# daxiongpro/EPNet

Measured on AMD Instinct MI355X. Metric: SA-stack points/sec per GPU (16384-pt KITTI scene) + % HBM roofline, higher is better.
Workload: dtype f32; 1 GPU; 256 x 16384-pt kitti scenes per GPU per step through the 4-level SA op stack (4 samplings [FPS + centre gather; levels 2-4 nested in level 1 where tie-free] + 8 ball_query + 8 fused groupings [xyz - centre ; features]), pyramid 16384>4096>1024>256>64, radii [[.1,.5],[.5,1],[1,2],[2,4]], nsample [16,32], C=0/96/256/512, HIP-graph launch; levels=4, scenes_per_gpu=256, software_pipelined=True, pipeline_stages=2, parallelism=scene-parallel x1

## Files before the change

epnet_amd/_lib.py:

```python
import ctypes
import os

_HERE = os.path.dirname(os.path.abspath(__file__))
LIB_PATH = os.environ.get("EPNET_HIP_LIB") or os.path.join(_HERE, "lib", "libepnet_hip.so")

_vp = ctypes.c_void_p
_i = ctypes.c_int
_f = ctypes.c_float
_sz = ctypes.c_size_t
_i64 = ctypes.c_int64

SIGNATURES = {
    "epnet_abi_version": (_i, []),
    "epnet_strerror": (ctypes.c_char_p, [_i]),
    "epnet_last_hip_error": (ctypes.c_char_p, []),
    "epnet_furthest_point_sampling": (_i, [_i, _i, _i, _vp, _vp, _vp, _vp]),
    "epnet_gather_points": (_i, [_i, _i, _i, _i, _vp, _vp, _vp, _vp]),
    "epnet_gather_points_grad": (_i, [_i, _i, _i, _i, _vp, _vp, _vp, _vp]),
    "epnet_ball_query": (_i, [_i, _i, _i, _f, _i, _vp, _vp, _vp, _vp]),
    "epnet_ball_query_workspace_bytes": (_sz, [_i, _i, _i]),
    "epnet_ball_query_ws": (_i, [_i, _i, _i, _f, _i, _vp, _vp, _vp, _vp, _sz, _vp]),
    "epnet_group_points": (_i, [_i, _i, _i, _i, _i, _vp, _vp, _vp, _vp]),
    "epnet_group_points_grad": (_i, [_i, _i, _i, _i, _i, _vp, _vp, _vp, _vp]),
    "epnet_group_concat": (_i, [_i, _i, _i, _i, _i, _vp, _vp, _vp, _vp, _vp, _i, _vp]),
# ... 5 lines not shown
    "epnet_group_concat_grad_ws": (_i, [_i, _i, _i, _i, _i, _vp, _vp, _vp, _i, _vp, _sz, _vp]),
    "epnet_three_nn": (_i, [_i, _i, _i, _vp, _vp, _vp, _vp, _vp]),
    "epnet_three_nn_workspace_bytes": (_sz, [_i, _i, _i]),
    "epnet_three_nn_ws": (_i, [_i, _i, _i, _vp, _vp, _vp, _vp, _vp, _sz, _vp]),
    "epnet_three_interpolate": (_i, [_i, _i, _i, _i, _vp, _vp, _vp, _vp, _vp]),
    "epnet_three_interpolate_grad": (_i, [_i, _i, _i, _i, _vp, _vp, _vp, _vp, _vp]),
    "epnet_three_interpolate_grad_workspace_bytes": (_sz, [_i, _i, _i]),
    "epnet_three_interpolate_grad_ws": (_i, [_i, _i, _i, _i, _vp, _vp, _vp, _vp, _vp, _sz, _vp]),
    "epnet_group_linear": (_i, [_i, _i, _i, _i, _i, _vp, _vp, _vp, _vp, _vp, _vp, _vp, _vp]),
    "epnet_group_linear_grad_w": (_i, [_i, _i, _i, _i, _i, _vp, _vp, _vp, _vp, _vp, _vp]),
    "epnet_feature_gather": (_i, [_i, _i, _i, _i, _i, _i, _i, _vp, _vp, _vp, _vp, _vp, _vp]),
    "epnet_feature_gather_grad": (_i, [_i, _i, _i, _i, _i, _i, _vp, _vp, _vp, _vp]),
    "epnet_pool_max": (_i, [ctypes.c_longlong, _i, _vp, _vp, _vp, _vp]),
    "epnet_pool_max_grad": (_i, [ctypes.c_longlong, _i, _vp, _vp, _vp, _vp]),
    "epnet_scene_index_bytes": (_sz, [_i, _i]),
    "epnet_scene_index_build": (_i, [_i, _i, _vp, _vp, _sz, _vp]),
    "epnet_scene_index_build_gathered": (_i, [_i, _i, _i, _vp, _vp, _vp, _vp, _sz, _vp]),
    "epnet_furthest_point_sampling_indexed": (_i, [_i, _i, _i, _vp, _vp, _sz, _vp, _vp, _vp]),
    "epnet_sample_centres": (_i, [_i, _i, _i, _vp, _vp, _sz, _vp, _vp, _vp, _vp]),
    "epnet_sample_centres_chain": (_i, [_i, _i, _i, _vp, _vp, _sz, _vp, _vp, _vp, _vp, _vp, _i, _vp]),
    "epnet_group_concat_multi": (_i, [_i, _i, _i, _i, _i, _vp, _vp, _vp, _vp, _vp, _vp, _i, _vp]),
    "epnet_ball_query_indexed_multi": (_i, [_i, _i, _i, _i, _vp, _vp, _vp, _vp, _vp, _sz, _vp, _vp]),
    "epnet_ball_query_ordered": (_i, [_i, _i, _i, _i, _vp, _vp, _vp, _vp, _vp, _sz, _vp, _sz, _vp, _vp]),
    "epnet_three_nn_indexed": (_i, [_i, _i, _i, _vp, _vp, _vp, _sz, _vp, _sz, _vp, _vp, _vp]),
    "epnet_ball_query_indexed": (_i, [_i, _i, _i, _f, _i, _vp, _vp, _vp, _sz, _vp, _vp]),
    "epnet_boxes_overlap_bev": (_i, [_i, _vp, _i, _vp, _vp, _vp]),
    "epnet_boxes_iou_bev": (_i, [_i, _vp, _i, _vp, _vp, _vp]),
    "epnet_boxes_iou3d": (_i, [_i, _vp, _i, _vp, _vp, _vp]),
    "epnet_boxes_iou3d_pairs": (_i, [_i, _vp, _vp, _vp, _vp]),
    "epnet_aug_roi_by_noise": (_i, [_i, _i, _f, _vp, _vp, _vp, _vp, _vp, _vp, _vp, _vp]),
    "epnet_rpn_proposals_workspace_bytes": (_sz, [_i, _i, _i, _i]),
    "epnet_rpn_proposals": (_i, [_i, _i, _vp, _vp, _vp, _i, _i, _i, _f, _i, _vp, _sz, _vp, _vp, _vp, _vp]),
    "epnet_nms_workspace_bytes": (_sz, [_i]),
    "epnet_nms": (_i, [_vp, _i, _f, _vp, _sz, _vp, _vp, _vp]),
    "epnet_nms_normal": (_i, [_vp, _i, _f, _vp, _sz, _vp, _vp, _vp]),
    "epnet_roipool3d_workspace_bytes": (_sz, [_i, _i, _i]),
    "epnet_roipool3d": (_i, [_i, _i, _i, _i, _i, _vp, _vp, _vp, _vp, _vp, _vp, _sz, _vp]),
    "epnet_pts_in_boxes3d_host": (_i, [_vp, _vp, _vp, _i64, _i64]),
    "epnet_roipool3d_host": (_i, [_vp, _vp, _vp, _vp, _vp, _vp, _i64, _i64, _i64, _i64]),
}

_lib = None


class EpnetError(RuntimeError):
    pass
# ... 30 lines not shown
```

epnet_amd/csrc/ball_query.hip:

```cpp
#include <stdlib.h>

#include "common.h"
#include "dpp.h"
#include "spatial.h"

namespace epnet {

constexpr int kBqTile = 2048;
constexpr int kBqThreads = 256;

template <int CPW>
__global__ __launch_bounds__(kBqThreads) void ball_query_kernel(int n, int m, float radius2, int nsample,
                                                                const float *__restrict__ new_xyz,
                                                                const float *__restrict__ xyz,
                                                                int *__restrict__ idx) {
    __shared__ float tile[kBqTile * 3];
    const int lane = threadIdx.x & 63, wave = threadIdx.x >> 6;
    const int bs = blockIdx.y;
    xyz += (size_t)bs * n * 3;
    new_xyz += (size_t)bs * m * 3;
    idx += (size_t)bs * m * nsample;

    const int c0 = (blockIdx.x * (kBqThreads / 64) + wave) * CPW;
    float cx[CPW], cy[CPW], cz[CPW];
// ... 325 lines not shown
        for (int q0 = 0; q0 < nq; q0 += 64) {
            const int qd = q0 + lane;
            const bool qnear = qd < nq && box_near(qboxes + qd * 6, cx, cy, cz, r2);
            const unsigned long long qmask = __ballot(qnear);
            if (!qmask) continue;
            const int nqc = (int)__popcll(qmask);
            if (qnear) quads[popc_below(qmask)] = qd;
            __builtin_amdgcn_wave_barrier();
            for (int s0 = 0; s0 < nqc; s0 += 16) {
                const int slot = s0 + (lane >> 2);
                int bid = 0;
                bool bnear = false;
                if (slot < nqc) {
                    bid = quads[slot] * 4 + (lane & 3);
                    bnear = box_near(boxes + bid * 6, cx, cy, cz, r2);
                }
                scan_buckets(__ballot(bnear), [&](int l) { return __builtin_amdgcn_readlane(bid, l); });
            }
            __builtin_amdgcn_wave_barrier();
        }
    }
}

__device__ __forceinline__ void bq_emit_list(int lane, const int *hits, int cnt, int nsample, int *__restrict__ out) {
    __builtin_amdgcn_wave_barrier();
    const int mine = lane < cnt ? hits[lane] : 0x7fffffff;
    int rank = 0;
    for (int j = 0; j < cnt; ++j) rank += __builtin_amdgcn_readlane(mine, j) < mine ? 1 : 0;
    if (lane < cnt && rank < nsample) out[rank] = mine;
    int first = 0;
    if (cnt) first = __builtin_amdgcn_readlane(mine, (int)__builtin_ctzll(__ballot(lane < cnt && rank == 0)));
    for (int l = cnt + lane; l < nsample; l += 64) out[l] = first;
}

template <int RM>
__device__ __forceinline__ int bq_select_smallest(int lane, int *hits, int cnt, int nsample, int np) {
    __builtin_amdgcn_wave_barrier();
    int key[RM];
#pragma unroll
    for (int r = 0; r < RM; ++r) key[r] = (r * 64 < cnt && r * 64 + lane < cnt) ? hits[r * 64 + lane] : 0x7fffffff;
    int lo = 0, hi = np;
    while (hi - lo > 1) {
        const int mid = (lo + hi) >> 1;
        int c = 0;
#pragma unroll
        for (int r = 0; r < RM; ++r)
            if (r * 64 < cnt) c += (int)__popcll(__ballot(key[r] < mid));
// ... 38 lines not shown
    if (bc > 0 && (pos < nsample || pos == 0)) {
        for (int i = 0; i < DPL; ++i) {
            unsigned ww = bits[lane * DPL + i];
            if (ww && mine_first == 0x7fffffff) mine_first = (lane * DPL + i) * 32 + (int)__builtin_ctz(ww);
            while (ww && pos < nsample) {
                const int bit = (int)__builtin_ctz(ww);
                ww &= ww - 1u;
                out[pos++] = (lane * DPL + i) * 32 + bit;
            }
            if (pos >= nsample) break;
        }
    }
    const unsigned long long have = __ballot(bc > 0);
    int first = 0;
    if (have) first = __builtin_amdgcn_readlane(mine_first, (int)__builtin_ctzll(have));
    for (int l = total + lane; l < nsample; l += 64) out[l] = first;
}

template <int K>
struct BqScales {
    float r2[K];
    int nsample[K];
    int *idx[K];
};

template <int DPL, int K>
__global__ __launch_bounds__(kQThreads) void bq_query_kernel(int np, int m, BqScales<K> sc,
                                                             const float *__restrict__ new_xyz,
                                                             const float4 *__restrict__ sorted,
                                                             const float *__restrict__ boxes,
                                                             const float *__restrict__ qboxes,
                                                             const float4 *__restrict__ order, int npc) {
    __shared__ unsigned s_bits[kQThreads / 64][64 * DPL];
    __shared__ int s_quads[kQThreads / 64][64];
    __shared__ int s_hits[kQThreads / 64][K][64];
    const int lane = threadIdx.x & 63, wave = threadIdx.x >> 6;
    int wg_x, bs;
    xcd_scene_map(wg_x, bs);
    int ci = wg_x * (kQThreads / 64) + wave;
    if (ci >= m) return;
    sorted += (size_t)bs * np;
    boxes += (size_t)bs * (np / 64) * 6;
    qboxes += (size_t)bs * (np / 256) * 6;
    float cx, cy, cz;
    if (order) {
        const float4 e = order[(size_t)bs * npc + ci];
        ci = __float_as_int(e.w);
// ... 12 lines not shown
        if (!__ballot(d2 < r2max)) return;
#pragma unroll
        for (int k = 0; k < K; ++k) {
            const bool hit = d2 < sc.r2[k];
            const unsigned long long hm = __ballot(hit);
            if (hm) {
                const int pos = cnt[k] + popc_below(hm);
                if (hit && pos < 64) s_hits[wave][k][pos] = __float_as_int(p.w);
                cnt[k] += (int)__popcll(hm);
            }
        }
    });
#pragma unroll
    for (int k = 0; k < K; ++k) {
        int *out = sc.idx[k] + ((size_t)bs * m + ci) * sc.nsample[k];
        if (cnt[k] <= 64)
            bq_emit_list(lane, s_hits[wave][k], cnt[k], sc.nsample[k], out);
        else
            bq_bitmap_search<DPL>(lane, np, sc.r2[k], sc.nsample[k], cx, cy, cz, sorted, boxes, qboxes, out, s_bits[wave],
                                  s_quads[wave]);
    }
}

template <int DPL, int K, bool kStream>
__global__ __launch_bounds__(kQThreads) void bq_query2_kernel(int np, int m, BqScales<K> sc,
                                                              const float *__restrict__ new_xyz,
                                                              const float4 *__restrict__ sorted,
                                                              const float *__restrict__ boxes,
                                                              const float *__restrict__ qboxes,
                                                              const float4 *__restrict__ order, int npc) {
    constexpr int CAP = kStream ? (K == 1 ? 512 : 256) : 64, kStepAppends = 128;
    constexpr int kBitWords = kStream ? 0 : 64 * DPL;
    __shared__ unsigned s_pool[kQThreads / 64][kBitWords + 2 * K * CAP];
    __shared__ int s_quads[kQThreads / 64][2][64];
    const int lane = threadIdx.x & 63, wave = threadIdx.x >> 6;
    int wg_x, bs;
    xcd_scene_map(wg_x, bs);
    const int ci0 = (wg_x * (kQThreads / 64) + wave) * 2;
    if (ci0 >= m) return;
    const bool two = ci0 + 1 < m;
    sorted += (size_t)bs * np;
    boxes += (size_t)bs * (np / 64) * 6;
    qboxes += (size_t)bs * (np / 256) * 6;
    float ax, ay, az, bx_, by_, bz_;
    int out0 = ci0, out1 = ci0 + 1;
    if (order) {
        const float4 e0 = order[(size_t)bs * npc + ci0], e1 = order[(size_t)bs * npc + ci0 + (two ? 1 : 0)];
        ax = e0.x; ay = e0.y; az = e0.z;
        bx_ = e1.x; by_ = e1.y; bz_ = e1.z;
        out0 = __float_as_int(e0.w);
        out1 = __float_as_int(e1.w);
    } else {
        const float *c0 = new_xyz + ((size_t)bs * m + ci0) * 3;
        const float *c1 = two ? c0 + 3 : c0;
        ax = c0[0]; ay = c0[1]; az = c0[2];
        bx_ = c1[0]; by_ = c1[1]; bz_ = c1[2];
// ... 96 lines not shown
                const int slot = s0 + ((lane & 31) >> 2);
                int bid = 0;
                bool bnear = false;
                if (slot < nmine) {
                    bid = s_quads[wave][half][slot] * 4 + (lane & 3);
                    bnear = box_near(boxes + bid * 6, hx, hy, hz, r2max);
                }
                const unsigned long long cand = __ballot(bnear);
                scan_pairs(cand & 0xFFFFFFFFull, cand >> 32,
                           [&](int e, int bit) { return __builtin_amdgcn_readlane(bid, bit + 32 * e); });
            }
            __builtin_amdgcn_wave_barrier();
        }
    }
#ifdef EPNET_BQ_STATS
    const unsigned long long st_1 = __builtin_amdgcn_s_memtime();
#endif
#pragma unroll
    for (int e = 0; e < 2; ++e) {
        if (e == 1 && !two) break;
        const float cx = e ? bx_ : ax, cy = e ? by_ : ay, cz = e ? bz_ : az;
#pragma unroll
        for (int k = 0; k < K; ++k) {
            int *out = sc.idx[k] + ((size_t)bs * m + (e ? out1 : out0)) * sc.nsample[k];
            int *hits = hits_of + (e * K + k) * CAP;
            if constexpr (kStream) {
                if (cnt[e][k] > 64) {
                    bq_select_smallest<CAP / 64>(lane, hits, cnt[e][k], sc.nsample[k], np);
                    cnt[e][k] = sc.nsample[k];
#ifdef EPNET_BQ_STATS
                    st_sel = true;
#endif
                }
                bq_emit_list(lane, hits, cnt[e][k], sc.nsample[k], out);
            } else {
                if (cnt[e][k] <= 64) {
                    bq_emit_list(lane, hits, cnt[e][k], sc.nsample[k], out);
                } else {
#ifdef EPNET_BQ_STATS
                    st_again = true;
#endif
                    bq_bitmap_search<DPL>(lane, np, sc.r2[k], sc.nsample[k], cx, cy, cz, sorted, boxes, qboxes, out, s_pool[wave],
                                          s_quads[wave][0]);
                }
            }
        }
    }
#ifdef EPNET_BQ_STATS
    {
        const unsigned long long st_3 = __builtin_amdgcn_s_memtime();
        if (lane == 0) {
            const int o = st_again ? 8 : (st_sel ? 4 : 0);
            atomicAdd(&g_bq_stats[o + 0], 1ull);
            atomicAdd(&g_bq_stats[o + 1], st_1 - st_0);
            atomicAdd(&g_bq_stats[o + 2], st_3 - st_1);
            atomicAdd(&g_bq_stats[o + 3], (unsigned long long)st_rows);
            atomicMax(&g_bq_stats[12], st_3 - st_0);
        }
    }
#endif
}

}

using namespace epnet;

extern "C" int epnet_ball_query(int b, int n, int m, float radius, int nsample, const float *new_xyz,
                                const float *xyz, int *idx, epnet_stream_t stream) {
    EPNET_REQUIRE(b >= 0 && n >= 0 && m >= 0 && nsample >= 0);
// ... 10 lines not shown
        dim3 grid(div_up(m, waves), b);
        hipLaunchKernelGGL(ball_query_kernel<1>, grid, dim3(kBqThreads), 0, s, n, m, radius2, nsample, new_xyz, xyz, idx);
    }
    return check_launch("ball_query");
}


int epnet::spatial_index_launch(int b, int n, int np, const float *xyz, float4 *sorted, float *boxes, float *qboxes,
                                hipStream_t s, int n_src, const int *src_idx, float *gathered) {
    if (n <= 4096) {
        constexpr int T = 256, cells = 1 << 12;
        const size_t stage = (np & 255) == 0 ? (size_t)(np / 4 < 512 ? np / 4 : 512) * sizeof(float4) : 0;
        hipLaunchKernelGGL((bq_index_kernel<T, 12>), dim3(b), dim3(T), (size_t)(cells + cells / (cells / T) + 64) * sizeof(int) + stage, s,
                           n, np, xyz, sorted, boxes, qboxes, n_src, src_idx, gathered);
    } else {
        constexpr int T = 1024, cells = 1 << 14;
        const size_t stage = (n <= T * 16 && (np & 255) == 0) ? (size_t)(np / 4) * sizeof(float4) : 0;
        hipLaunchKernelGGL((bq_index_kernel<T, 14>), dim3(b), dim3(T), (size_t)(cells + cells / (cells / T) + 64) * sizeof(int) + stage, s,
                           n, np, xyz, sorted, boxes, qboxes, n_src, src_idx, gathered);
    }
    return check_launch("spatial index");
}

template <int K>
static int bq_query_launch(int b, int np, int m, const BqScales<K> &sc, const float *new_xyz, const float4 *sorted,
                           hipStream_t s, const float4 *order = nullptr, int npc = 0) {
    const float *boxes = (const float *)(sorted + (size_t)b * np);
    const float *qboxes = boxes + (size_t)b * (np / 64) * 6;
    const char *pair_str = getenv("EPNET_BQ_PAIR");
    const int pair_env = pair_str ? atoi(pair_str) : -1;
    const bool pair = pair_env >= 0 ? pair_env != 0 : (long long)b * m >= 65536;
    const char *pad_str = getenv("EPNET_BQ_PAD_KB");
    const size_t pad = pad_str ? (size_t)atoi(pad_str) * 1024 : 0;
    if (pair) {
        dim3 grid(div_up(div_up(m, 2), kQThreads / 64), b);
        bool stream = np > 16384;
        if (const char *e = getenv("EPNET_BQ_STREAM")) stream = atoi(e) != 0;
        for (int k = 0; k < K; ++k) stream = stream && sc.nsample[k] <= 64;
#define EPNET_BQ2(D_)                                                                                                                   \
    do {                                                                                                                                \
        if (stream)                                                                                                                     \
            hipLaunchKernelGGL((bq_query2_kernel<D_, K, true>), grid, dim3(kQThreads), pad, s, np, m, sc, new_xyz, sorted, boxes, qboxes, \
                               order, npc);                                                                                             \
        else                                                                                                                            \
            hipLaunchKernelGGL((bq_query2_kernel<D_, K, false>), grid, dim3(kQThreads), pad, s, np, m, sc, new_xyz, sorted, boxes,       \
                               qboxes, order, npc);                                                                                     \
    } while (0)
        switch (np / 2048) {
            case 1: EPNET_BQ2(1); break;
            case 2: EPNET_BQ2(2); break;
            case 4: EPNET_BQ2(4); break;
            case 8: EPNET_BQ2(8); break;
            case 16: EPNET_BQ2(16); break;
            default: EPNET_BQ2(32); break;
        }
#undef EPNET_BQ2
        return check_launch("ball_query query");
    }
    dim3 grid(div_up(m, kQThreads / 64), b);
#define EPNET_BQ(D_) hipLaunchKernelGGL((bq_query_kernel<D_, K>), grid, dim3(kQThreads), pad, s, np, m, sc, new_xyz, sorted, boxes, qboxes, order, npc)
    switch (np / 2048) {
        case 1: EPNET_BQ(1); break;
        case 2: EPNET_BQ(2); break;
        case 4: EPNET_BQ(4); break;
        case 8: EPNET_BQ(8); break;
        case 16: EPNET_BQ(16); break;
        default: EPNET_BQ(32); break;
    }
#undef EPNET_BQ
    return check_launch("ball_query query");
}

extern "C" size_t epnet_scene_index_bytes(int b, int n) { return scene_index_bytes(b, n); }

extern "C" int epnet_scene_index_build(int b, int n, const float *xyz, void *index, size_t index_bytes,
                                       epnet_stream_t stream) {
    const size_t need = scene_index_bytes(b, n);
    EPNET_REQUIRE(need != 0 && xyz && index);
    if (index_bytes < need) return EPNET_ENOMEM;
// ... 39 lines not shown
extern "C" int epnet_ball_query_indexed_multi(int b, int n, int m, int nscales, const float *radii, const int *nsamples,
                                              const float *new_xyz, const float *xyz, const void *index,
                                              size_t index_bytes, int *const *idx, epnet_stream_t stream) {
    EPNET_REQUIRE(nscales >= 0 && (nscales == 0 || (radii && nsamples && idx)));
    const size_t need = scene_index_bytes(b, n);
    bool fused = nscales == 2 && need != 0 && index && m > 0 && nsamples[0] > 0 && nsamples[1] > 0;
    if (!fused) {
        for (int k = 0; k < nscales; ++k) {
            const int rc = epnet_ball_query_indexed(b, n, m, radii[k], nsamples[k], new_xyz, xyz, index, index_bytes, idx[k], stream);
            if (rc) return rc;
        }
        return EPNET_OK;
    }
    EPNET_REQUIRE(new_xyz && idx[0] && idx[1]);
    if (index_bytes < need) return EPNET_ENOMEM;
    EPNET_REQUIRE(b <= 65535);
    BqScales<2> sc;
    for (int k = 0; k < 2; ++k) {
        sc.r2[k] = radii[k] * radii[k];
        sc.nsample[k] = nsamples[k];
        sc.idx[k] = idx[k];
    }
    return bq_query_launch<2>(b, scene_index_np(n), m, sc, new_xyz, (const float4 *)index, (hipStream_t)stream);
}

extern "C" int epnet_ball_query_ordered(int b, int n, int m, int nscales, const float *radii, const int *nsamples,
                                        const float *new_xyz, const float *xyz, const void *index, size_t index_bytes,
                                        const void *centre_index, size_t centre_index_bytes, int *const *idx,
                                        epnet_stream_t stream) {
    EPNET_REQUIRE(nscales >= 0 && (nscales == 0 || (radii && nsamples && idx)));
    const size_t need = scene_index_bytes(b, n), need_c = scene_index_bytes(b, m);
    bool ordered = (nscales == 1 || nscales == 2) && need != 0 && need_c != 0 && index && centre_index && m > 0;
    for (int k = 0; ordered && k < nscales; ++k) ordered = nsamples[k] > 0 && idx[k] != nullptr;
    const char *force = getenv("EPNET_BQ_ORDERED");
    if (force ? atoi(force) == 0 : n <= 16384) ordered = false;
    if (!ordered) return epnet_ball_query_indexed_multi(b, n, m, nscales, radii, nsamples, new_xyz, xyz, index, index_bytes, idx, stream);
    if (index_bytes < need || centre_index_bytes < need_c) return EPNET_ENOMEM;
    EPNET_REQUIRE(b <= 65535);
    const int np = scene_index_np(n), npc = scene_index_np(m);
    if (nscales == 1) {
        BqScales<1> sc;
        sc.r2[0] = radii[0] * radii[0];
        sc.nsample[0] = nsamples[0];
        sc.idx[0] = idx[0];
        return bq_query_launch<1>(b, np, m, sc, new_xyz, (const float4 *)index, (hipStream_t)stream, (const float4 *)centre_index, npc);
    }
// ... 42 lines not shown
```

epnet_amd/csrc/common.h:

```cpp
#pragma once
#include <hip/hip_runtime.h>
#include <stdint.h>

#include "epnet_ops.h"

namespace epnet {

constexpr int kWave = 64;

int record_hip_error(hipError_t e, const char *where);

inline int check_launch(const char *where) {
    hipError_t e = hipGetLastError();
    if (e != hipSuccess) return record_hip_error(e, where);
    return EPNET_OK;
}

inline int div_up(int a, int b) { return (a + b - 1) / b; }
inline long long div_up64(long long a, long long b) { return (a + b - 1) / b; }

__device__ __forceinline__ int lane_id() { return threadIdx.x & (kWave - 1); }

__device__ __forceinline__ int popc_below(unsigned long long mask) {
    return __builtin_amdgcn_mbcnt_hi((unsigned)(mask >> 32), __builtin_amdgcn_mbcnt_lo((unsigned)mask, 0));
}

__device__ __forceinline__ void store_stream(float *dst, float x, float y, float z, float w) {
    typedef float f4 __attribute__((ext_vector_type(4)));
    const f4 v = {x, y, z, w};
    __builtin_nontemporal_store(v, reinterpret_cast<f4 *>(dst));
}

__device__ __forceinline__ void xcd_scene_map(int &wg_x, int &bs) {
#ifdef EPNET_NO_XCD_MAP
    wg_x = (int)blockIdx.x;
    bs = (int)blockIdx.y;
#else
    const int gx = (int)gridDim.x, nwg = gx * (int)gridDim.y, orig = (int)blockIdx.y * gx + (int)blockIdx.x;
    const int xcd = orig & 7, qq = nwg >> 3, rr = nwg & 7;
    const int wgid = (xcd < rr ? xcd * (qq + 1) : rr * (qq + 1) + (xcd - rr) * qq) + (orig >> 3);
    bs = wgid / gx;
    wg_x = wgid - bs * gx;
// ... 33 lines not shown
```

epnet_amd/csrc/group.hip:

```cpp
#include <stdlib.h>

#include "common.h"
#include "spatial.h"
#include "runsum.h"

namespace epnet {

constexpr int kGThreads = 256;
constexpr int kGChan = 16;

__global__ __launch_bounds__(kGThreads) void gather_rows_vec4_kernel(int c, int n, int p, size_t ostride,
                                                                     const float *__restrict__ points,
                                                                     const int *__restrict__ idx,
                                                                     float *__restrict__ out) {
    int wg_x, wg_y, bs;
    xcd_scene_map3(wg_x, wg_y, bs);
    const int c0 = wg_y * kGChan;
    const int q4 = wg_x * kGThreads + threadIdx.x;
    if (q4 * 4 >= p) return;
    const int4 id = *reinterpret_cast<const int4 *>(idx + (size_t)bs * p + (size_t)q4 * 4);
    const int cend = min(c, c0 + kGChan);
    const float *src = points + ((size_t)bs * c + c0) * n;
    float *dst = out + (size_t)bs * ostride + (size_t)c0 * p + (size_t)q4 * 4;
#pragma unroll 4
// ... 568 lines not shown
    return launch_gather_rows(b, c, n, npoints, points, idx, out, (hipStream_t)stream, "gather_points");
}

extern "C" int epnet_gather_points_grad(int b, int c, int n, int npoints, const float *grad_out, const int *idx,
                                        float *grad_points, epnet_stream_t stream) {
    EPNET_REQUIRE(b >= 0 && c >= 0 && n >= 0 && npoints >= 0);
    return launch_scatter_rows(b, c, n, npoints, grad_out, idx, grad_points, (hipStream_t)stream, "gather_points_grad");
}

extern "C" int epnet_group_points(int b, int c, int n, int npoints, int nsample, const float *points, const int *idx,
                                  float *out, epnet_stream_t stream) {
    EPNET_REQUIRE(b >= 0 && c >= 0 && n >= 0 && npoints >= 0 && nsample >= 0);
    return launch_gather_rows(b, c, n, (long long)npoints * nsample, points, idx, out, (hipStream_t)stream,
                              "group_points");
}

extern "C" int epnet_group_points_grad(int b, int c, int n, int npoints, int nsample, const float *grad_out,
                                       const int *idx, float *grad_points, epnet_stream_t stream) {
    EPNET_REQUIRE(b >= 0 && c >= 0 && n >= 0 && npoints >= 0 && nsample >= 0);
    return launch_scatter_rows(b, c, n, (long long)npoints * nsample, grad_out, idx, grad_points, (hipStream_t)stream,
                               "group_points_grad");
}

static int launch_group_xyz(int b, int n, int npoints, int nsample, long long p, size_t ostride, const float *xyz,
                            const float *new_xyz, const int *idx, float *out, hipStream_t s) {
    if (nsample % 4 == 0 && (((uintptr_t)idx | (uintptr_t)out) % 16 == 0) && (ostride % 4 == 0))
        hipLaunchKernelGGL(group_xyz_centred_vec4_kernel, dim3((unsigned)div_up64(p / 4, kGThreads), b), dim3(kGThreads), 0, s, n,
                           npoints, nsample, ostride, xyz, new_xyz, idx, out);
    else
        hipLaunchKernelGGL(group_xyz_centred_kernel, dim3((unsigned)div_up64(p, kGThreads), b), dim3(kGThreads), 0, s, n, npoints,
                           nsample, ostride, xyz, new_xyz, idx, out);
    return check_launch("group_concat xyz");
}

extern "C" int epnet_group_concat(int b, int c, int n, int npoints, int nsample, const float *xyz, const float *new_xyz,
                                  const float *features, const int *idx, float *out, int use_xyz, epnet_stream_t stream) {
    EPNET_REQUIRE(b >= 0 && c >= 0 && n >= 0 && npoints >= 0 && nsample >= 0);
    EPNET_REQUIRE(use_xyz || c > 0);
    const long long p = (long long)npoints * nsample;
    if (b == 0 || p == 0) return EPNET_OK;
    EPNET_REQUIRE(idx && out && (c == 0 || features) && (!use_xyz || (xyz && new_xyz)));
    EPNET_REQUIRE(n > 0);
    if (p > 0x7fffffffll || b > 65535) return EPNET_ELIMIT;
    hipStream_t s = (hipStream_t)stream;
    const int ch0 = use_xyz ? 3 : 0;
    const size_t ostride = (size_t)(ch0 + c) * (size_t)p;
    if (use_xyz) {
// ... 184 lines not shown
```

epnet_amd/pointnet2_cuda.py:

```python
import torch

from . import _lib
from ._tensor import dev_ptr, need, on_device_of, writes

_F, _I = torch.float32, torch.int32


@writes("idx")
def ball_query_wrapper(b, n, m, radius, nsample, new_xyz, xyz, idx):
    pn, px, pi = dev_ptr(new_xyz, "new_xyz", _F), dev_ptr(xyz, "xyz", _F), dev_ptr(idx, "idx", _I)
    need(new_xyz, b * m * 3, "new_xyz"); need(xyz, b * n * 3, "xyz"); need(idx, b * m * nsample, "idx")
    l = _lib.lib()
    ws_bytes = l.epnet_ball_query_workspace_bytes(b, n, m)
    with on_device_of(xyz) as s:
        if ws_bytes:
            ws = torch.empty((ws_bytes,), dtype=torch.uint8, device=xyz.device)
            _lib.check(l.epnet_ball_query_ws(b, n, m, radius, nsample, pn, px, pi, ws.data_ptr(), ws_bytes, s), "ball_query")
        else:
            _lib.check(l.epnet_ball_query(b, n, m, radius, nsample, pn, px, pi, s), "ball_query")
    return 1


@writes("out")
def group_points_wrapper(b, c, n, npoints, nsample, points, idx, out):
# ... 182 lines not shown
                       "sample_centres")
    return 1


@writes("idxs")
def ball_query_multi_wrapper(b, n, m, radii, nsamples, new_xyz, xyz, index, idxs):
    import ctypes
    pn, pxyz = dev_ptr(new_xyz, "new_xyz", _F), dev_ptr(xyz, "xyz", _F)
    need(new_xyz, b * m * 3, "new_xyz"); need(xyz, b * n * 3, "xyz")
    k = len(radii)
    assert len(nsamples) == k and len(idxs) == k
    ptrs = []
    for ns, t in zip(nsamples, idxs):
        ptrs.append(dev_ptr(t, "idx", _I))
        need(t, b * m * ns, "idx")
    px, nb = _index_args(index, xyz)
    c_r = (ctypes.c_float * k)(*[float(r) for r in radii])
    c_n = (ctypes.c_int * k)(*[int(x) for x in nsamples])
    c_p = (ctypes.c_void_p * k)(*ptrs)
    with on_device_of(xyz) as s:
        _lib.check(_lib.lib().epnet_ball_query_indexed_multi(b, n, m, k, ctypes.cast(c_r, ctypes.c_void_p),
                                                             ctypes.cast(c_n, ctypes.c_void_p), pn, pxyz, px, nb,
                                                             ctypes.cast(c_p, ctypes.c_void_p), s), "ball_query")
    return 1


@writes("idxs")
def ball_query_ordered_wrapper(b, n, m, radii, nsamples, new_xyz, xyz, index, centre_index, idxs):
    import ctypes
    pn, pxyz = dev_ptr(new_xyz, "new_xyz", _F), dev_ptr(xyz, "xyz", _F)
    need(new_xyz, b * m * 3, "new_xyz"); need(xyz, b * n * 3, "xyz")
    k = len(radii)
    assert len(nsamples) == k and len(idxs) == k
    ptrs = []
    for ns, t in zip(nsamples, idxs):
        ptrs.append(dev_ptr(t, "idx", _I))
        need(t, b * m * ns, "idx")
    px, nb = _index_args(index, xyz)
    pc, nc = _index_args(centre_index, new_xyz)
    c_r = (ctypes.c_float * k)(*[float(r) for r in radii])
    c_n = (ctypes.c_int * k)(*[int(x) for x in nsamples])
    c_p = (ctypes.c_void_p * k)(*ptrs)
    with on_device_of(xyz) as s:
        _lib.check(_lib.lib().epnet_ball_query_ordered(b, n, m, k, ctypes.cast(c_r, ctypes.c_void_p), ctypes.cast(c_n, ctypes.c_void_p),
                                                     pn, pxyz, px, nb, pc, nc, ctypes.cast(c_p, ctypes.c_void_p), s), "ball_query")
    return 1
# ... 166 lines not shown
```

epnet_amd/sa_stack.py:

```python
import os

import torch

from . import pointnet2_cuda as ext

RPN_NPOINTS = (4096, 1024, 256, 64)
RPN_RADII = ((0.1, 0.5), (0.5, 1.0), (1.0, 2.0), (2.0, 4.0))
RPN_NSAMPLES = ((16, 32), (16, 32), (16, 32), (16, 32))
RPN_FEAT_CHANNELS = (0, 96, 256, 512)
RPN_FP = ((1024, 64, 256), (512, 256, 1024), (512, 1024, 4096), (256, 4096, 16384))


CONFIGS = {
    2: dict(n=16384, npoints=RPN_NPOINTS, radii=RPN_RADII, nsamples=RPN_NSAMPLES, feat_channels=RPN_FEAT_CHANNELS),
    5: dict(n=65536, npoints=(16384,), radii=((0.5,),), nsamples=((64,),), feat_channels=(64,)),
}


def sa_algorithmic_bytes(n=16384, npoints=RPN_NPOINTS, nsamples=RPN_NSAMPLES, feat_channels=RPN_FEAT_CHANNELS):
    out = {"fps": 0, "gather": 0, "ball_query": 0, "group_xyz": 0, "group_feat": 0}
    cur = n
    for lvl, m in enumerate(npoints):
        out["fps"] += cur * 12 + m * 4
        out["gather"] += m * 4 + 3 * cur * 4 + 3 * m * 4
# ... 40 lines not shown
            chosen = frozenset(int(v) for v in s_query_levels)
        elif queries_in_s is not None:
            chosen = every if queries_in_s else frozenset()
        elif env_lv is not None:
            chosen = frozenset(int(v) for v in env_lv.split(",") if v.strip())
        elif self.stages == 3:
            chosen = every
        elif env_q == 2 or (env_q == 1 and with_fp):
            chosen = every
        elif env_q == 1 and batch * n >= 240 * 16384:
            chosen = every - {0}
        else:
            chosen = frozenset()
        self.s_query_levels = chosen & every
        self.queries_in_s = self.s_query_levels == every
        self.chain = bool(int(os.environ.get("EPNET_SA_CHAIN", "1"))) and fused_sampling
        self.fuse_gather = bool(int(os.environ.get("EPNET_SA_FUSE_GATHER", "1")))
        self._deferred = None
        self.s_first = bool(int(os.environ.get("EPNET_SA_S_FIRST", "0" if self.s_query_levels else "1")))
        self.tail_scales = int(os.environ.get("EPNET_SA_TAIL_SCALES", "0"))
        self.multi_query = bool(int(os.environ.get("EPNET_SA_MULTI_QUERY", "1")))
        self.multi_group = bool(int(os.environ.get("EPNET_SA_MULTI_GROUP", "1")))
        self.ordered_query = bool(int(os.environ.get("EPNET_SA_ORDERED_QUERY", "1")))
        self.side = None
        self.npoints, self.radii, self.nsamples, self.feat_channels = npoints, radii, nsamples, feat_channels
        self.with_fp, self.fp = with_fp, fp
        dev = torch.device(device)
        g = torch.Generator().manual_seed(seed)
        f32, i32 = torch.float32, torch.int32
        self.levels = []
        cur = n
        for lvl, m in enumerate(npoints):
            c = feat_channels[lvl]
            index_bytes = ext.scene_index_bytes(batch, cur) if shared_index else 0
            L = {
                "n": cur, "m": m, "c": c,
                "xyz_t_sets": [torch.empty((batch, 3, cur), dtype=f32, device=dev) for _ in range(self.ring if not fused else 1)],
                "temp": torch.empty((batch, cur), dtype=f32, device=dev),
                "fps_idx_sets": ([torch.empty((batch, m), dtype=i32, device=dev) for _ in range(3)] if self.stages == 3 else None),
                "fps_idx": None,
                "new_xyz_t": torch.empty((batch, 3, m), dtype=f32, device=dev),
                "sets": [{"new_xyz": torch.empty((batch, m, 3), dtype=f32, device=dev),
                          "index": (torch.empty((index_bytes,), dtype=torch.uint8, device=dev) if index_bytes else None),
                          "prefix": torch.zeros((batch,), dtype=i32, device=dev),
                          "centre_index": (torch.empty((ext.scene_index_bytes(batch, m),), dtype=torch.uint8, device=dev)
                                           if (shared_index and lvl + 1 == len(npoints) and ext.scene_index_bytes(batch, m)) else None)}
# ... 141 lines not shown
        else:
            for S in L["scales"]:
                self._query_scale(L, S, cur_xyz, parity)

    def _centre_index(self, L, parity):
        lvl = self.levels.index(L)
        if lvl + 1 < len(self.levels):
            return self.levels[lvl + 1]["sets"][parity]["index"] if self.shared_index else None
        own = L["sets"][parity].get("centre_index")
        if own is not None:
            ext.scene_index_build_wrapper(self.batch, L["m"], L["sets"][parity]["new_xyz"], own)
        return own

    def _group_scales(self, L, cur_xyz, parity):
        if self.fused and self.multi_group and len(L["scales"]) > 1:
            ext.group_concat_multi_wrapper(self.batch, L["c"], L["n"], L["m"], [S["ns"] for S in L["scales"]], cur_xyz,
                                           L["sets"][parity]["new_xyz"], L["features"], [self._idx(S, parity) for S in L["scales"]],
                                           [S["grouped"] for S in L["scales"]], True)
        else:
            for S in L["scales"]:
                self._group_scale(L, S, cur_xyz, parity)

    def _group_level(self, L, cur_xyz, parity):
        self._query_level(L, cur_xyz, parity)
        self._group_scales(L, cur_xyz, parity)

    def _side_stream(self, device):
        if self.side is None:
            self.side = torch.cuda.Stream(device=device)
        return self.side

    def run(self, xyz):
        main = torch.cuda.current_stream(xyz.device)
        side = self._side_stream(xyz.device) if self.overlap else None
        cur_xyz = xyz
        built = False
        for lvl, L in enumerate(self.levels):
            new_xyz = self._sample_level(L, cur_xyz, 0, index_built=built)
            built = False
            nxt = self.levels[lvl + 1] if lvl + 1 < len(self.levels) else None
            if self.ordered_query and L["n"] > 16384 and nxt is not None and nxt["sets"][0]["index"] is not None:
                ext.scene_index_build_wrapper(self.batch, L["m"], new_xyz, nxt["sets"][0]["index"])
                built = True
            if side is not None:
                side.wait_stream(main)
                with torch.cuda.stream(side):
# ... 209 lines not shown
```

include/epnet_ops.h:

```cpp
#ifndef EPNET_OPS_H
#define EPNET_OPS_H

#include <stddef.h>
#include <stdint.h>

#ifdef __cplusplus
extern "C" {
#endif

#define EPNET_ABI_VERSION 1

#define EPNET_OK 0
#define EPNET_EINVAL (-1)
#define EPNET_ELAUNCH (-2)
#define EPNET_ENOMEM (-3)
#define EPNET_ELIMIT (-4)

typedef void *epnet_stream_t;

int epnet_abi_version(void);
const char *epnet_strerror(int code);
const char *epnet_last_hip_error(void);


// ... 72 lines not shown
                         const float *xy, const int *idx, float *out, float *xy_out, epnet_stream_t stream);
int epnet_feature_gather_grad(int b, int c, int h, int w, int n, int align_corners, const float *grad_out, const float *xy,
                              float *grad_feature_map, epnet_stream_t stream);

size_t epnet_scene_index_bytes(int b, int n);
int epnet_scene_index_build(int b, int n, const float *xyz, void *index, size_t index_bytes, epnet_stream_t stream);
int epnet_scene_index_build_gathered(int b, int n_src, int n, const float *xyz_src, const int *idx, float *gathered, void *index,
                                     size_t index_bytes, epnet_stream_t stream);
int epnet_furthest_point_sampling_indexed(int b, int n, int m, const float *xyz, void *index,
                                          size_t index_bytes, float *temp, int *idx, epnet_stream_t stream);
int epnet_sample_centres(int b, int n, int m, const float *xyz, void *index, size_t index_bytes, float *temp,
                         int *idx, float *new_xyz, epnet_stream_t stream);
int epnet_sample_centres_chain(int b, int n, int m, const float *xyz, void *index, size_t index_bytes, float *temp,
                               int *idx, float *new_xyz, const int *prefix_in, int *prefix_out, int prefix_cap,
                               epnet_stream_t stream);
int epnet_three_nn_indexed(int b, int n, int m, const float *unknown, const float *known, const void *unknown_index,
                           size_t unknown_index_bytes, const void *known_index, size_t known_index_bytes, float *dist2,
                           int *idx, epnet_stream_t stream);
int epnet_ball_query_indexed(int b, int n, int m, float radius, int nsample, const float *new_xyz, const float *xyz,
                             const void *index, size_t index_bytes, int *idx, epnet_stream_t stream);
int epnet_ball_query_indexed_multi(int b, int n, int m, int nscales, const float *radii, const int *nsamples,
                                   const float *new_xyz, const float *xyz, const void *index, size_t index_bytes,
                                   int *const *idx, epnet_stream_t stream);
int epnet_ball_query_ordered(int b, int n, int m, int nscales, const float *radii, const int *nsamples, const float *new_xyz,
                             const float *xyz, const void *index, size_t index_bytes, const void *centre_index,
                             size_t centre_index_bytes, int *const *idx, epnet_stream_t stream);


int epnet_boxes_overlap_bev(int num_a, const float *boxes_a, int num_b, const float *boxes_b,
                            float *ans_overlap, epnet_stream_t stream);

int epnet_boxes_iou_bev(int num_a, const float *boxes_a, int num_b, const float *boxes_b,
                        float *ans_iou, epnet_stream_t stream);

int epnet_boxes_iou3d(int num_a, const float *boxes_a, int num_b, const float *boxes_b, float *ans_iou3d,
                      epnet_stream_t stream);

int epnet_boxes_iou3d_pairs(int k, const float *boxes_a, const float *boxes_b, float *ans_iou3d, epnet_stream_t stream);

int epnet_aug_roi_by_noise(int k, int aug_times, float pos_thresh, float *roi_boxes3d, const float *gt_boxes3d,
                           const float *iou3d_src, const int *tries, const unsigned char *keep_draw,
                           const float *noise, float *iou_of_rois, epnet_stream_t stream);

size_t epnet_rpn_proposals_workspace_bytes(int b, int distance_based, int pre_nms_top_n, int post_nms_top_n);
int epnet_rpn_proposals(int b, int n, const float *proposals, const float *scores, const int64_t *order,
                        int distance_based, int pre_nms_top_n, int post_nms_top_n, float nms_thresh, int rotated,
// ... 32 lines not shown
```

Before: 1.323 billion points/s.

## Fuse centred xyz grouping into the paired ball-query kernel for C=0 levels

```diff
diff --git a/epnet_amd/_lib.py b/epnet_amd/_lib.py
--- a/epnet_amd/_lib.py
+++ b/epnet_amd/_lib.py
@@ -51,6 +51,7 @@
     "epnet_group_concat_multi": (_i, [_i, _i, _i, _i, _i, _vp, _vp, _vp, _vp, _vp, _vp, _i, _vp]),
     "epnet_ball_query_indexed_multi": (_i, [_i, _i, _i, _i, _vp, _vp, _vp, _vp, _vp, _sz, _vp, _vp]),
     "epnet_ball_query_ordered": (_i, [_i, _i, _i, _i, _vp, _vp, _vp, _vp, _vp, _sz, _vp, _sz, _vp, _vp]),
+    "epnet_ball_query_group_xyz": (_i, [_i, _i, _i, _i, _vp, _vp, _vp, _vp, _vp, _sz, _i, _vp, _vp, _vp]),
     "epnet_three_nn_indexed": (_i, [_i, _i, _i, _vp, _vp, _vp, _sz, _vp, _sz, _vp, _vp, _vp]),
     "epnet_ball_query_indexed": (_i, [_i, _i, _i, _f, _i, _vp, _vp, _vp, _sz, _vp, _vp]),
     "epnet_boxes_overlap_bev": (_i, [_i, _vp, _i, _vp, _vp, _vp]),
diff --git a/epnet_amd/csrc/ball_query.hip b/epnet_amd/csrc/ball_query.hip
--- a/epnet_amd/csrc/ball_query.hip
+++ b/epnet_amd/csrc/ball_query.hip
@@ -371,7 +371,7 @@
     }
 }
 
-__device__ __forceinline__ void bq_emit_list(int lane, const int *hits, int cnt, int nsample, int *__restrict__ out) {
+__device__ __forceinline__ void bq_emit_list(int lane, const int *hits, int cnt, int nsample, int *out) {
     __builtin_amdgcn_wave_barrier();
     const int mine = lane < cnt ? hits[lane] : 0x7fffffff;
     int rank = 0;
@@ -456,7 +456,53 @@
     float r2[K];
     int nsample[K];
     int *idx[K];
+    float *grp[K];
+    unsigned long long gstride[K];
 };
+
+template <int V, int K>
+__device__ __forceinline__ void bq_write_rows(int lane, const BqScales<K> &sc, const int *hits_of, int cap, bool two, int bs, int m,
+                                              int row0, int row1, float ax, float ay, float az, float bx, float by, float bz,
+                                              const float *__restrict__ xyz, int n) {
+    const int u0 = sc.nsample[0] / V, u1 = K > 1 ? sc.nsample[K - 1] / V : 0, per_centre = u0 + u1;
+    const int total = two ? 2 * per_centre : per_centre;
+    const float *base = xyz + (size_t)bs * n * 3;
+    for (int f = lane; f < total; f += 64) {
+        int g = f;
+        const bool e = g >= per_centre;
+        g = e ? g - per_centre : g;
+        const bool k1 = K > 1 && g >= u0;
+        g = k1 ? g - u0 : g;
+        const int ns = k1 ? sc.nsample[K - 1] : sc.nsample[0];
+        int *idx = k1 ? sc.idx[K - 1] : sc.idx[0];
+        float *grp = k1 ? sc.grp[K - 1] : sc.grp[0];
+        const size_t gstride = k1 ? sc.gstride[K - 1] : sc.gstride[0];
+        const int row = e ? row1 : row0;
+        const float cx = e ? bx : ax, cy = e ? by : ay, cz = e ? bz : az;
+        const int *src = hits_of + ((e ? K : 0) + (k1 ? 1 : 0)) * cap + g * V;
+        const size_t p = (size_t)m * ns, o = (size_t)row * ns + (size_t)g * V;
+        float *dst = grp + (size_t)bs * gstride + o;
+        if constexpr (V == 4) {
+            const int4 id = *reinterpret_cast<const int4 *>(src);
+            *reinterpret_cast<int4 *>(idx + (size_t)bs * p + o) = id;
+            const float *p0 = base + (size_t)id.x * 3, *p1 = base + (size_t)id.y * 3, *p2 = base + (size_t)id.z * 3,
+                        *p3 = base + (size_t)id.w * 3;
+            const float x0 = p0[0], y0 = p0[1], z0 = p0[2], x1 = p1[0], y1 = p1[1], z1 = p1[2];
+            const float x2 = p2[0], y2 = p2[1], z2 = p2[2], x3 = p3[0], y3 = p3[1], z3 = p3[2];
+            store_stream(dst, x0 - cx, x1 - cx, x2 - cx, x3 - cx);
+            store_stream(dst + p, y0 - cy, y1 - cy, y2 - cy, y3 - cy);
+            store_stream(dst + 2 * p, z0 - cz, z1 - cz, z2 - cz, z3 - cz);
+        } else {
+            const int id = *src;
+            idx[(size_t)bs * p + o] = id;
+            const float *pt = base + (size_t)id * 3;
+            const float x = pt[0], y = pt[1], z = pt[2];
+            dst[0] = x - cx;
+            dst[p] = y - cy;
+            dst[2 * p] = z - cz;
+        }
+    }
+}
 
 template <int DPL, int K>
 __global__ __launch_bounds__(kQThreads) void bq_query_kernel(int np, int m, BqScales<K> sc,
@@ -515,16 +561,17 @@
     }
 }
 
-template <int DPL, int K, bool kStream>
+template <int DPL, int K, bool kStream, int kXyz>
 __global__ __launch_bounds__(kQThreads) void bq_query2_kernel(int np, int m, BqScales<K> sc,
                                                               const float *__restrict__ new_xyz,
                                                               const float4 *__restrict__ sorted,
                                                               const float *__restrict__ boxes,
                                                               const float *__restrict__ qboxes,
-                                                              const float4 *__restrict__ order, int npc) {
+                                                              const float4 *__restrict__ order, int npc,
+                                                              const float *__restrict__ xyz, int n) {
     constexpr int CAP = kStream ? (K == 1 ? 512 : 256) : 64, kStepAppends = 128;
     constexpr int kBitWords = kStream ? 0 : 64 * DPL;
-    __shared__ unsigned s_pool[kQThreads / 64][kBitWords + 2 * K * CAP];
+    __shared__ __attribute__((aligned(16))) unsigned s_pool[kQThreads / 64][kBitWords + 2 * K * CAP];
     __shared__ int s_quads[kQThreads / 64][2][64];
     const int lane = threadIdx.x & 63, wave = threadIdx.x >> 6;
     int wg_x, bs;
@@ -667,8 +714,8 @@
         const float cx = e ? bx_ : ax, cy = e ? by_ : ay, cz = e ? bz_ : az;
 #pragma unroll
         for (int k = 0; k < K; ++k) {
-            int *out = sc.idx[k] + ((size_t)bs * m + (e ? out1 : out0)) * sc.nsample[k];
             int *hits = hits_of + (e * K + k) * CAP;
+            int *out = kXyz ? hits : sc.idx[k] + ((size_t)bs * m + (e ? out1 : out0)) * sc.nsample[k];
             if constexpr (kStream) {
                 if (cnt[e][k] > 64) {
                     bq_select_smallest<CAP / 64>(lane, hits, cnt[e][k], sc.nsample[k], np);
@@ -690,6 +737,10 @@
                 }
             }
         }
+    }
+    if constexpr (kXyz != 0) {
+        __builtin_amdgcn_wave_barrier();
+        bq_write_rows<kXyz, K>(lane, sc, hits_of, CAP, two, bs, m, out0, out1, ax, ay, az, bx_, by_, bz_, xyz, n);
     }
 #ifdef EPNET_BQ_STATS
     {
@@ -746,14 +797,19 @@
     return check_launch("spatial index");
 }
 
+static bool bq_pair(int b, int m) {
+    const char *pair_str = getenv("EPNET_BQ_PAIR");
+    const int pair_env = pair_str ? atoi(pair_str) : -1;
+    return pair_env >= 0 ? pair_env != 0 : (long long)b * m >= 65536;
+}
+
 template <int K>
 static int bq_query_launch(int b, int np, int m, const BqScales<K> &sc, const float *new_xyz, const float4 *sorted,
-                           hipStream_t s, const float4 *order = nullptr, int npc = 0) {
+                           hipStream_t s, const float4 *order = nullptr, int npc = 0, const float *xyz = nullptr, int n = 0,
+                           int vec = 0) {
     const float *boxes = (const float *)(sorted + (size_t)b * np);
     const float *qboxes = boxes + (size_t)b * (np / 64) * 6;
-    const char *pair_str = getenv("EPNET_BQ_PAIR");
-    const int pair_env = pair_str ? atoi(pair_str) : -1;
-    const bool pair = pair_env >= 0 ? pair_env != 0 : (long long)b * m >= 65536;
+    const bool pair = xyz || bq_pair(b, m);
     const char *pad_str = getenv("EPNET_BQ_PAD_KB");
     const size_t pad = pad_str ? (size_t)atoi(pad_str) * 1024 : 0;
     if (pair) {
@@ -761,14 +817,19 @@
         bool stream = np > 16384;
         if (const char *e = getenv("EPNET_BQ_STREAM")) stream = atoi(e) != 0;
         for (int k = 0; k < K; ++k) stream = stream && sc.nsample[k] <= 64;
-#define EPNET_BQ2(D_)                                                                                                                   \
-    do {                                                                                                                                \
-        if (stream)                                                                                                                     \
-            hipLaunchKernelGGL((bq_query2_kernel<D_, K, true>), grid, dim3(kQThreads), pad, s, np, m, sc, new_xyz, sorted, boxes, qboxes, \
-                               order, npc);                                                                                             \
-        else                                                                                                                            \
-            hipLaunchKernelGGL((bq_query2_kernel<D_, K, false>), grid, dim3(kQThreads), pad, s, np, m, sc, new_xyz, sorted, boxes,       \
-                               qboxes, order, npc);                                                                                     \
+#define EPNET_BQ2X(D_, S_, X_)                                                                                                       \
+    hipLaunchKernelGGL((bq_query2_kernel<D_, K, S_, X_>), grid, dim3(kQThreads), pad, s, np, m, sc, new_xyz, sorted, boxes, qboxes, \
+                       order, npc, xyz, n)
+#define EPNET_BQ2S(D_, S_)                          \
+    do {                                            \
+        if (!xyz) EPNET_BQ2X(D_, S_, 0);            \
+        else if (vec == 4) EPNET_BQ2X(D_, S_, 4);   \
+        else EPNET_BQ2X(D_, S_, 1);                 \
+    } while (0)
+#define EPNET_BQ2(D_)                      \
+    do {                                   \
+        if (stream) EPNET_BQ2S(D_, true);  \
+        else EPNET_BQ2S(D_, false);        \
     } while (0)
         switch (np / 2048) {
             case 1: EPNET_BQ2(1); break;
@@ -779,6 +840,8 @@
             default: EPNET_BQ2(32); break;
         }
 #undef EPNET_BQ2
+#undef EPNET_BQ2S
+#undef EPNET_BQ2X
         return check_launch("ball_query query");
     }
     dim3 grid(div_up(m, kQThreads / 64), b);
@@ -864,6 +927,51 @@
         sc.idx[k] = idx[k];
     }
     return bq_query_launch<2>(b, scene_index_np(n), m, sc, new_xyz, (const float4 *)index, (hipStream_t)stream);
+}
+
+extern "C" int epnet_ball_query_group_xyz(int b, int n, int m, int nscales, const float *radii, const int *nsamples,
+                                          const float *new_xyz, const float *xyz, const void *index, size_t index_bytes, int c,
+                                          int *const *idx, float *const *grouped, epnet_stream_t stream) {
+    EPNET_REQUIRE(b >= 0 && n >= 0 && m >= 0 && c >= 0 && nscales >= 0 && (nscales == 0 || (radii && nsamples && idx && grouped)));
+    if (b == 0 || m == 0) return EPNET_OK;
+    EPNET_REQUIRE(new_xyz && xyz && n > 0);
+    const size_t need = scene_index_bytes(b, n);
+    bool fused = (nscales == 1 || nscales == 2) && need != 0 && index && index_bytes >= need && b <= 65535 && bq_pair(b, m);
+    bool vec4 = true;
+    for (int k = 0; k < nscales; ++k) {
+        EPNET_REQUIRE(nsamples[k] >= 0 && idx[k] && grouped[k]);
+        if ((long long)m * nsamples[k] > 0x7fffffffll) return EPNET_ELIMIT;
+        fused = fused && nsamples[k] > 0 && nsamples[k] <= 64;
+        vec4 = vec4 && nsamples[k] % 4 == 0 && (((uintptr_t)idx[k] | (uintptr_t)grouped[k]) % 16) == 0;
+    }
+    hipStream_t s = (hipStream_t)stream;
+    if (!fused) {
+        int rc = epnet_ball_query_indexed_multi(b, n, m, nscales, radii, nsamples, new_xyz, xyz, index, index_bytes, idx, stream);
+        for (int k = 0; k < nscales && rc == EPNET_OK; ++k) {
+            const long long p = (long long)m * nsamples[k];
+            if (p) rc = launch_group_xyz(b, n, m, nsamples[k], p, (size_t)(3 + c) * (size_t)p, xyz, new_xyz, idx[k], grouped[k], s);
+        }
+        return rc;
+    }
+    const int np = scene_index_np(n);
+    if (nscales == 1) {
+        BqScales<1> sc;
+        sc.r2[0] = radii[0] * radii[0];
+        sc.nsample[0] = nsamples[0];
+        sc.idx[0] = idx[0];
+        sc.grp[0] = grouped[0];
+        sc.gstride[0] = (unsigned long long)(3 + c) * m * nsamples[0];
+        return bq_query_launch<1>(b, np, m, sc, new_xyz, (const float4 *)index, s, nullptr, 0, xyz, n, vec4 ? 4 : 1);
+    }
+    BqScales<2> sc;
+    for (int k = 0; k < 2; ++k) {
+        sc.r2[k] = radii[k] * radii[k];
+        sc.nsample[k] = nsamples[k];
+        sc.idx[k] = idx[k];
+        sc.grp[k] = grouped[k];
+        sc.gstride[k] = (unsigned long long)(3 + c) * m * nsamples[k];
+    }
+    return bq_query_launch<2>(b, np, m, sc, new_xyz, (const float4 *)index, s, nullptr, 0, xyz, n, vec4 ? 4 : 1);
 }
 
 extern "C" int epnet_ball_query_ordered(int b, int n, int m, int nscales, const float *radii, const int *nsamples,
diff --git a/epnet_amd/csrc/common.h b/epnet_amd/csrc/common.h
--- a/epnet_amd/csrc/common.h
+++ b/epnet_amd/csrc/common.h
@@ -18,6 +18,9 @@
 
 inline int div_up(int a, int b) { return (a + b - 1) / b; }
 inline long long div_up64(long long a, long long b) { return (a + b - 1) / b; }
+
+int launch_group_xyz(int b, int n, int npoints, int nsample, long long p, size_t ostride, const float *xyz, const float *new_xyz,
+                     const int *idx, float *out, hipStream_t s);
 
 __device__ __forceinline__ int lane_id() { return threadIdx.x & (kWave - 1); }
 
diff --git a/epnet_amd/csrc/group.hip b/epnet_amd/csrc/group.hip
--- a/epnet_amd/csrc/group.hip
+++ b/epnet_amd/csrc/group.hip
@@ -614,7 +614,7 @@
                                "group_points_grad");
 }
 
-static int launch_group_xyz(int b, int n, int npoints, int nsample, long long p, size_t ostride, const float *xyz,
+int epnet::launch_group_xyz(int b, int n, int npoints, int nsample, long long p, size_t ostride, const float *xyz,
                             const float *new_xyz, const int *idx, float *out, hipStream_t s) {
     if (nsample % 4 == 0 && (((uintptr_t)idx | (uintptr_t)out) % 16 == 0) && (ostride % 4 == 0))
         hipLaunchKernelGGL(group_xyz_centred_vec4_kernel, dim3((unsigned)div_up64(p / 4, kGThreads), b), dim3(kGThreads), 0, s, n,
diff --git a/epnet_amd/pointnet2_cuda.py b/epnet_amd/pointnet2_cuda.py
--- a/epnet_amd/pointnet2_cuda.py
+++ b/epnet_amd/pointnet2_cuda.py
@@ -228,6 +228,30 @@
         _lib.check(_lib.lib().epnet_ball_query_indexed_multi(b, n, m, k, ctypes.cast(c_r, ctypes.c_void_p),
                                                              ctypes.cast(c_n, ctypes.c_void_p), pn, pxyz, px, nb,
                                                              ctypes.cast(c_p, ctypes.c_void_p), s), "ball_query")
+    return 1
+
+
+@writes("idxs", "grouped")
+def ball_query_multi_group_xyz_wrapper(b, n, m, radii, nsamples, new_xyz, xyz, index, c, idxs, grouped):
+    import ctypes
+    pn, pxyz = dev_ptr(new_xyz, "new_xyz", _F), dev_ptr(xyz, "xyz", _F)
+    need(new_xyz, b * m * 3, "new_xyz"); need(xyz, b * n * 3, "xyz")
+    k = len(radii)
+    assert len(nsamples) == k and len(idxs) == k and len(grouped) == k
+    ptrs, gptrs = [], []
+    for ns, t, g in zip(nsamples, idxs, grouped):
+        ptrs.append(dev_ptr(t, "idx", _I))
+        gptrs.append(dev_ptr(g, "grouped", _F))
+        need(t, b * m * ns, "idx"); need(g, b * (3 + c) * m * ns, "grouped")
+    px, nb = _index_args(index, xyz)
+    c_r = (ctypes.c_float * k)(*[float(r) for r in radii])
+    c_n = (ctypes.c_int * k)(*[int(x) for x in nsamples])
+    c_p = (ctypes.c_void_p * k)(*ptrs)
+    c_g = (ctypes.c_void_p * k)(*gptrs)
+    with on_device_of(xyz) as s:
+        _lib.check(_lib.lib().epnet_ball_query_group_xyz(b, n, m, k, ctypes.cast(c_r, ctypes.c_void_p), ctypes.cast(c_n, ctypes.c_void_p),
+                                                       pn, pxyz, px, nb, int(c), ctypes.cast(c_p, ctypes.c_void_p),
+                                                       ctypes.cast(c_g, ctypes.c_void_p), s), "ball_query")
     return 1
 
 
diff --git a/epnet_amd/sa_stack.py b/epnet_amd/sa_stack.py
--- a/epnet_amd/sa_stack.py
+++ b/epnet_amd/sa_stack.py
@@ -86,6 +86,7 @@
         self.multi_query = bool(int(os.environ.get("EPNET_SA_MULTI_QUERY", "1")))
         self.multi_group = bool(int(os.environ.get("EPNET_SA_MULTI_GROUP", "1")))
         self.ordered_query = bool(int(os.environ.get("EPNET_SA_ORDERED_QUERY", "1")))
+        self.query_groups_xyz = bool(int(os.environ.get("EPNET_SA_QUERY_XYZ", "1")))
         self.side = None
         self.npoints, self.radii, self.nsamples, self.feat_channels = npoints, radii, nsamples, feat_channels
         self.with_fp, self.fp = with_fp, fp
@@ -273,6 +274,13 @@
                 self._group_scale(L, S, cur_xyz, parity)
 
     def _group_level(self, L, cur_xyz, parity):
+        P = L["sets"][parity]
+        if (self.query_groups_xyz and self.fused and self.multi_query and L["c"] == 0 and P["index"] is not None
+                and not (self.ordered_query and L["n"] > 16384)):
+            ext.ball_query_multi_group_xyz_wrapper(self.batch, L["n"], L["m"], [S["radius"] for S in L["scales"]],
+                                             [S["ns"] for S in L["scales"]], P["new_xyz"], cur_xyz, P["index"], 0,
+                                             [self._idx(S, parity) for S in L["scales"]], [S["grouped"] for S in L["scales"]])
+            return
         self._query_level(L, cur_xyz, parity)
         self._group_scales(L, cur_xyz, parity)
 
diff --git a/include/epnet_ops.h b/include/epnet_ops.h
--- a/include/epnet_ops.h
+++ b/include/epnet_ops.h
@@ -118,6 +118,9 @@
 int epnet_ball_query_indexed_multi(int b, int n, int m, int nscales, const float *radii, const int *nsamples,
                                    const float *new_xyz, const float *xyz, const void *index, size_t index_bytes,
                                    int *const *idx, epnet_stream_t stream);
+int epnet_ball_query_group_xyz(int b, int n, int m, int nscales, const float *radii, const int *nsamples, const float *new_xyz,
+                               const float *xyz, const void *index, size_t index_bytes, int c, int *const *idx,
+                               float *const *grouped, epnet_stream_t stream);
 int epnet_ball_query_ordered(int b, int n, int m, int nscales, const float *radii, const int *nsamples, const float *new_xyz,
                              const float *xyz, const void *index, size_t index_bytes, const void *centre_index,
                              size_t centre_index_bytes, int *const *idx, epnet_stream_t stream);
diff --git a/profiles/micro/bq_xyz_bench.py b/profiles/micro/bq_xyz_bench.py
--- /dev/null
+++ b/profiles/micro/bq_xyz_bench.py
@@ -0,0 +1,37 @@
+import sys
+sys.path.insert(0, '.')
+import torch
+from epnet_amd import pointnet2_cuda as ext, synth
+dev = 'cuda:0'
+b = int(sys.argv[1]) if len(sys.argv) > 1 else 256
+n, m, radii, nss = 16384, 4096, [0.1, 0.5], [16, 32]
+xyz = torch.stack([synth.kitti_like_cloud(n, 3 + i) for i in range(b)]).to(dev)
+g = torch.Generator().manual_seed(0)
+rows = torch.stack([torch.randperm(n, generator=g)[:m] for _ in range(b)]).to(dev)
+centres = torch.gather(xyz, 1, rows[..., None].expand(b, m, 3)).contiguous()
+index = ext.scene_index(xyz)
+idxs = [torch.empty((b, m, ns), dtype=torch.int32, device=dev) for ns in nss]
+grouped = [torch.empty((b, 3, m, ns), dtype=torch.float32, device=dev) for ns in nss]
+
+
+def composition():
+    ext.ball_query_multi_wrapper(b, n, m, radii, nss, centres, xyz, index, idxs)
+    for ns, idx, out in zip(nss, idxs, grouped):
+        ext.group_concat_wrapper(b, 0, n, m, ns, xyz, centres, None, idx, out, True)
+
+
+def fused():
+    ext.ball_query_multi_group_xyz_wrapper(b, n, m, radii, nss, centres, xyz, index, 0, idxs, grouped)
+
+
+for name, fn in (("composition", composition), ("fused", fused), ("composition", composition), ("fused", fused)):
+    for _ in range(3):
+        fn()
+    torch.cuda.synchronize()
+    e0, e1 = torch.cuda.Event(enable_timing=True), torch.cuda.Event(enable_timing=True)
+    e0.record()
+    for _ in range(20):
+        fn()
+    e1.record()
+    torch.cuda.synchronize()
+    print("%-11s scenes %d: %.4f ms per call" % (name, b, e0.elapsed_time(e1) / 20))
```

Measured after the change: 1.344 billion points/s (median of 6 runs). 1.7% higher.
